# LIS-TU-Berlin/SVN-ICP

Measured on AMD Instinct MI355X. Metric: scan-pair registrations/sec at N particles x M source pts, 1/2/4/8 GPU, higher is better.
Workload: dtype f64; 1 GPU; C3: 128 particles SVN-ICP, 131072-pt source vs 262144-pt target, K=100, I=20, max_dist=1.0, lr=1.0, SVNFullGrad=False, correspondence=fast, early stop off; synthetic 64-beam scans (seed 20250718); particles=128, target_points=262144, knn_count=100, parallelism=single GPU

## Files before the change

svn-icp_amd/csrc/particle_update.hip:

```cpp
#include "kernels.hpp"
#include "update_single.hpp"
#include "stein_split_device.hpp"

namespace svnicp {

namespace {

constexpr int UT = 512;
constexpr int KREG = 32;

struct Work {
  double *H, *b, *N, *x, *phi, *sq;
  __device__ Work(double* w, int P) {
    H = w; b = H + (size_t)P * 36; N = b + (size_t)P * 6; x = N + (size_t)P * 6; phi = x + (size_t)P * 6;
    sq = phi + (size_t)P * 6;
  }
};

__device__ __forceinline__ void load_sums(const UpdateArgs& a, int p, double* s) {
  const double* rec = a.sums + (size_t)p * kNSums;
  const size_t stride = a.sums_stride ? (size_t)a.sums_stride : (size_t)a.P * kNSums;
#pragma unroll
  for (int i = 0; i < kNSums; ++i) s[i] = rec[i];
  for (int r = 1; r < a.n_ranks; ++r) {
// ... 1249 lines not shown
    r[0] = init[3 * P + p]; r[1] = init[4 * P + p]; r[2] = init[5 * P + p];
    tv[0] = init[p]; tv[1] = init[P + p]; tv[2] = init[2 * P + p];
    if (mode == 0) so3_exp(r, Rm, nullptr); else euler_to_R(r[0], r[1], r[2], Rm);
    if (mode == 1 && eul) {
      for (int i = 0; i < 3; ++i) { eul[6 * p + i] = tv[i]; eul[6 * p + 3 + i] = r[i]; }
    }
  }
  double Rt[9], tt[3];
  mat3_mul(pose.R0, Rm, Rt);
  mat3_vec(pose.R0, tv, tt);
  for (int i = 0; i < 9; ++i) { R[9 * p + i] = Rm[i]; Rtot[12 * p + i] = Rt[i]; }
  for (int i = 0; i < 3; ++i) { t[3 * p + i] = tv[i]; Rtot[12 * p + 9 + i] = pose.t0[i] + tt[i]; }
  if (refresh_pose) {
    double lg[3];
    if (mode == 0) so3_log(Rm, lg); else { lg[0] = r[0]; lg[1] = r[1]; lg[2] = r[2]; }
    for (int i = 0; i < 3; ++i) { pose_out[i * P + p] = tv[i]; pose_out[(3 + i) * P + p] = lg[i]; }
  }
}

__global__ void k_stats(StatsArgs a) {
  const int tid = threadIdx.x;
  const int P = a.P;
  __shared__ double mean[6];
  constexpr int kStage = 1024;
  __shared__ double sp[6 * kStage];
  const bool staged = P <= kStage;
  if (staged) for (int e = tid; e < 6 * P; e += blockDim.x) sp[e] = a.pose[e];
  __syncthreads();
  const double* pose = staged ? sp : a.pose;
  const double wsvn = (double)(1.0f / (float)P);
  if (tid < 6) {
    double s = 0.0;
    if (a.mode == 0) { for (int p = 0; p < P; ++p) s += pose[tid * P + p] * wsvn; }
    else { for (int p = 0; p < P; ++p) s += pose[tid * P + p]; s /= P; }
    mean[tid] = s;
    a.out[tid] = s;
  }
  __syncthreads();
  if (tid < 6) {
    double s = 0.0;
    if (a.mode == 0) { for (int p = 0; p < P; ++p) { const double d = pose[tid * P + p] - mean[tid]; s += d * d * wsvn; } }
    else { for (int p = 0; p < P; ++p) { const double d = pose[tid * P + p] - mean[tid]; s += d * d; } s /= (P - 1); }
    a.out[6 + tid] = s;
  }
  if (tid < 36) {
    const int r = tid / 6, c = tid % 6;
    double s = 0.0;
    const double wgt = a.mode == 0 ? wsvn : 1.0;
    for (int p = 0; p < P; ++p) s += wgt * ((pose[r * P + p] - mean[r]) * (pose[c * P + p] - mean[c]));
    a.out[12 + tid] = a.mode == 0 ? s : s / P;
  }
  for (int p = tid; p < P; p += blockDim.x) a.out[48 + p] = a.mode == 0 ? wsvn : 1.0;
}

}

size_t update_workspace_doubles(int P) { return (size_t)P * (36 + 6 * 4) + (size_t)P * P + 64; }
size_t update_uctl_doubles(int P) { return (size_t)UCTL_NORM + (size_t)((P + 7) & ~7) + (size_t)HB_NB / 2 + (size_t)36 * ((P + 127) / 128) + 8; }

hipError_t launch_init_particles(const double* init6xP, int P, const Pose0& pose, int mode, double* R, double* t,
                                 double* Rtot, double* pose_out, int refresh_pose, double* eul, hipStream_t st, const BeginZero* zero) {
  BeginZero z{};
  if (zero) z = *zero;
  unsigned int most = 0;
  for (int a = 0; a < z.n; ++a) most = z.dwords[a] > most ? z.dwords[a] : most;
  int blocks = (P + 127) / 128;
  const int for_zero = (int)((most + 128u * 32u - 1u) / (128u * 32u));
  if (for_zero > blocks) blocks = for_zero > 256 ? 256 : for_zero;
  hipLaunchKernelGGL(k_init_particles, dim3(blocks), dim3(128), 0, st, init6xP, P, pose, mode, R, t, Rtot,
                     pose_out, refresh_pose, eul, z);
  return hipGetLastError();
}

hipError_t launch_update_median(const UpdateArgs& a, int num_cus, int max_p_one_workgroup, hipStream_t st) {
  const int P = a.P;
  if (P <= max_p_one_workgroup && P <= 128) {
    const size_t smem = (size_t)P * 6 * sizeof(double) + (size_t)(FRONT_BUF + 8) * sizeof(double) + (size_t)HB_NB * sizeof(unsigned int);
    hipError_t e = hipFuncSetAttribute(reinterpret_cast<const void*>(k_upd_median), hipFuncAttributeMaxDynamicSharedMemorySize, (int)smem);
    if (e != hipSuccess) return e;
    hipLaunchKernelGGL(k_upd_median, dim3(1), dim3(UT), smem, st, a);
    return hipGetLastError();
  }
  const size_t n = (size_t)P * P;
  const size_t xs = (size_t)P * 6 * sizeof(double);
  int nb = (int)((n + 1023) / 1024);
  if (nb > num_cus / 2) nb = num_cus / 2;
  if (nb < 1) nb = 1;
  const size_t lds_hist = xs + (size_t)HB_NB * sizeof(unsigned int);
  const size_t lds_coll = xs + (size_t)COLL_CHUNK * sizeof(double);
  const size_t lds_sel = (size_t)SEL_LDS_KEYS * sizeof(double);
  if (lds_hist > 150 * 1024 || lds_coll > 150 * 1024) return hipErrorInvalidValue;
  {
    hipError_t e = hipFuncSetAttribute(reinterpret_cast<const void*>(k_upd_hist), hipFuncAttributeMaxDynamicSharedMemorySize, 150 * 1024);
    if (e == hipSuccess) e = hipFuncSetAttribute(reinterpret_cast<const void*>(k_upd_collect), hipFuncAttributeMaxDynamicSharedMemorySize, 150 * 1024);
    if (e == hipSuccess) e = hipFuncSetAttribute(reinterpret_cast<const void*>(k_upd_select), hipFuncAttributeMaxDynamicSharedMemorySize, (int)lds_sel);
    if (e != hipSuccess) return e;
  }
  hipLaunchKernelGGL(k_upd_hist, dim3(nb), dim3(256), lds_hist, st, a);
  hipLaunchKernelGGL(k_upd_collect, dim3(nb), dim3(256), lds_coll, st, a);
  hipLaunchKernelGGL(k_upd_select, dim3(1), dim3(UT), lds_sel, st, a);
  return hipGetLastError();
}

hipError_t launch_update_prepare(const UpdateArgs& a, hipStream_t st) {
  const int need_mean = (!a.svgd && !a.full_grad) ? 1 : 0;
  hipLaunchKernelGGL(k_upd_prepare, dim3((a.P + PREP_PW - 1) / PREP_PW + need_mean), dim3(PREP_T), 0, st, a);
  return hipGetLastError();
}

hipError_t launch_update_prepare_median(const UpdateArgs& a, hipStream_t st) {
  const int P = a.P;
  const int need_mean = (!a.svgd && !a.full_grad) ? 1 : 0;
  const size_t smem = (size_t)P * 6 * sizeof(double) + (size_t)(FRONT_BUF + 8) * sizeof(double) + (size_t)HB_NB * sizeof(unsigned int);
  hipError_t e = hipFuncSetAttribute(reinterpret_cast<const void*>(k_upd_prepare_median), hipFuncAttributeMaxDynamicSharedMemorySize, (int)smem);
  if (e != hipSuccess) return e;
  hipLaunchKernelGGL(k_upd_prepare_median, dim3((P + PREP_PW - 1) / PREP_PW + need_mean + 1), dim3(UT), smem, st, a);
  return hipGetLastError();
}

namespace {
template <int PW, int WP, int NRB, bool TAIL>
hipError_t launch_small_t(const AccumArgs& a, const UpdateArgs& u, const SmallArgs& s, int grid, size_t smem, hipStream_t st) {
  const void* fn = u.svgd ? reinterpret_cast<const void*>(k_small_registration<PW, WP, NRB, TAIL, true>)
                          : reinterpret_cast<const void*>(k_small_registration<PW, WP, NRB, TAIL, false>);
  hipError_t e = hipFuncSetAttribute(fn, hipFuncAttributeMaxDynamicSharedMemorySize, (int)smem);
  if (e != hipSuccess) return e;
  int per_cu = 0;
  e = hipOccupancyMaxActiveBlocksPerMultiprocessor(&per_cu, fn, 256, smem);
  if (e != hipSuccess) return e;
  if (per_cu < 1) return hipErrorCooperativeLaunchTooLarge;
  AccumArgs aa = a; UpdateArgs uu = u; SmallArgs ss = s;
  void* args[3] = {&aa, &uu, &ss};
  return hipLaunchCooperativeKernel(fn, dim3((unsigned)grid), dim3(256), args, (unsigned int)smem, st);
}
}

bool small_registration_supported(int PW, int WP, int K) {
  return K >= 97 && K <= 100 && ((WP == 1 && (PW == 16 || PW == 32 || PW == 64)) || (PW == 64 && WP == 2));
}

hipError_t launch_small_registration(const AccumPlan& plan, AccumArgs a, const UpdateArgs& u, int iterations, unsigned int* bar,
                                     int num_cus, hipStream_t st) {
  const int P = u.P;
  a.Ppad = plan.Ppad; a.pts_per_block = plan.pts_per_block; a.spts_per_block = plan.pts_per_block;
  SmallArgs s{};
  s.GA = plan.grid_x; s.iterations = iterations; s.bar = bar;
  {
    const int pass = 4 * (64 / plan.PW);
    int64_t spb = (a.B + (num_cus - 2)) / (num_cus - 1);
    spb = (spb + pass - 1) / pass * pass;
    s.spts_per_block = (int)spb;
    s.GS = (int)((a.B + spb - 1) / spb);
  }
  const int n_prep = (P + PREP_PW - 1) / PREP_PW + ((!u.svgd && !u.full_grad) ? 1 : 0);
  const int n_dir = (P + 3) / 4;
  int grid = s.GS + 1;
  if (s.GA > grid) grid = s.GA;
  if (n_prep > grid) grid = n_prep;
  if (n_dir > grid) grid = n_dir;
  if (grid > num_cus) return hipErrorCooperativeLaunchTooLarge;
  const size_t smem_median = (size_t)P * 6 * sizeof(double) + (size_t)(FRONT_BUF + 8) * sizeof(double) + (size_t)HB_NB * sizeof(unsigned int);
  const size_t smem = smem_median > plan.smem ? smem_median : plan.smem;
  if (!small_registration_supported(plan.PW, plan.WP, plan.K)) return hipErrorInvalidValue;
  if (plan.PW == 16) return launch_small_t<16, 1, 6, true>(a, u, s, grid, smem, st);
  if (plan.PW == 32) return launch_small_t<32, 1, 6, true>(a, u, s, grid, smem, st);
  if (plan.WP == 1) return launch_small_t<64, 1, 6, true>(a, u, s, grid, smem, st);
  return launch_small_t<64, 2, 6, true>(a, u, s, grid, smem, st);
}

hipError_t launch_update_direction(const UpdateArgs& a, hipStream_t st, bool finish) {
  hipLaunchKernelGGL(k_upd_direction, dim3((a.P + 3) / 4), dim3(256), 0, st, a);
  if (finish && (a.check_early_stop || a.trH)) hipLaunchKernelGGL(k_upd_finish, dim3(1), dim3(256), 0, st, a);
  return hipGetLastError();
}
const double* update_step_norms(const UpdateArgs& a) { return a.uctl + UCTL_NORM; }

hipError_t launch_reduce_partials(const double* partial, int nblk, int Ppad, int p_lo, int n_particles, double* sums, const int* ctl,
                                  hipStream_t st) {
  const int n_entries = n_particles * kNSums;
  if (n_entries <= 0) return hipSuccess;
  hipLaunchKernelGGL(k_reduce_partials, dim3((n_entries + 15) / 16), dim3(256), 0, st, partial, nblk, Ppad, p_lo, n_particles, sums, ctl);
  return hipGetLastError();
}

hipError_t launch_update(const UpdateArgs& a_in, hipStream_t st) {
  UpdateArgs a = a_in;
  const size_t base = (size_t)a.P * 24 * sizeof(double);
  const size_t with_h = base + (size_t)a.P * 36 * sizeof(double);
  a.h_in_lds = with_h <= 120 * 1024 ? 1 : 0;
  const size_t smem = a.h_in_lds ? with_h : base;
  if (smem > 150 * 1024) return hipErrorInvalidValue;
  if (smem > 64 * 1024) {
    hipError_t e = hipFuncSetAttribute(reinterpret_cast<const void*>(k_particle_update),
                                       hipFuncAttributeMaxDynamicSharedMemorySize, (int)smem);
    if (e != hipSuccess) return e;
  }
  hipLaunchKernelGGL(k_particle_update, dim3(1), dim3(UT), smem, st, a);
  return hipGetLastError();
}

hipError_t launch_update_svgd(const UpdateArgs& a, hipStream_t st) {
  const size_t smem = (size_t)a.P * 18 * sizeof(double);
  if (smem > 150 * 1024) return hipErrorInvalidValue;
  if (smem > 64 * 1024) {
    hipError_t e = hipFuncSetAttribute(reinterpret_cast<const void*>(k_particle_update_svgd),
                                       hipFuncAttributeMaxDynamicSharedMemorySize, (int)smem);
    if (e != hipSuccess) return e;
  }
  hipLaunchKernelGGL(k_particle_update_svgd, dim3(1), dim3(UT), smem, st, a);
  return hipGetLastError();
}

hipError_t launch_stats(const StatsArgs& a, hipStream_t st) {
  hipLaunchKernelGGL(k_stats, dim3(1), dim3(256), 0, st, a);
  return hipGetLastError();
}

}
```

svn-icp_amd/csrc/stein_split.hip:

```cpp
#include "stein_split_device.hpp"

namespace svnicp {

namespace {

constexpr float kSentinelCC = 1.0e30f;
__global__ __launch_bounds__(256) void k_build_table3(const int32_t* __restrict__ idx, int64_t B, int K,
                                                      const double* __restrict__ tgt, int64_t M, double* __restrict__ table,
                                                      double* __restrict__ anchor, float4* __restrict__ tablea,
                                                      float* __restrict__ cmax) {
  __shared__ float rowbuf[4][128 * 4];
  const int lane = threadIdx.x & (kWave - 1), wave = threadIdx.x >> 6;
  const int64_t b = (int64_t)blockIdx.x * 4 + wave;
  if (b >= B) return;
  int64_t i0 = idx[b * K];
  i0 = i0 < 0 ? 0 : (i0 >= M ? M - 1 : i0);
  const double a0 = tgt[3 * i0], a1 = tgt[3 * i0 + 1], a2 = tgt[3 * i0 + 2];
  float cm = 0.0f;
  float* rb = rowbuf[wave];
  for (int k = lane; k < 128; k += kWave) {
    float cx = 0.f, cy = 0.f, cz = 0.f, cc = kSentinelCC;
    if (k < K) {
      int64_t i = idx[b * K + k];
      i = i < 0 ? 0 : (i >= M ? M - 1 : i);
      const double x = tgt[3 * i], y = tgt[3 * i + 1], z = tgt[3 * i + 2];
      if (table) {
        double* o = table + ((size_t)b * K + k) * 3;
        o[0] = x; o[1] = y; o[2] = z;
      }
      cx = (float)(x - a0); cy = (float)(y - a1); cz = (float)(z - a2);
      cc = (float)(((double)cx * cx + (double)cy * cy) + (double)cz * cz);
      cm = __builtin_fmaxf(cm, (float)sqrt(((double)cx * cx + (double)cy * cy) + (double)cz * cz) * 1.0000002f);
      if (!(cc < kSentinelCC)) cm = __builtin_nanf("");
    }
    rb[4 * k] = cx; rb[4 * k + 1] = cy; rb[4 * k + 2] = cz; rb[4 * k + 3] = cc;
  }
  for (int off = 32; off > 0; off >>= 1) {
    const float o = __shfl_xor(cm, off, kWave);
    cm = (cm != cm || o != o) ? __builtin_nanf("") : __builtin_fmaxf(cm, o);
  }
  if (lane == 0) {
    cmax[b] = cm;
    anchor[3 * b] = a0; anchor[3 * b + 1] = a1; anchor[3 * b + 2] = a2;
  }
  __builtin_amdgcn_wave_barrier();
  const int mi = lane & 15, mk = lane >> 4;
#pragma unroll
  for (int h = 0; h < 2; ++h) {
    float4 v;
    v.x = rb[4 * (16 * (4 * h + 0) + mi) + mk];
    v.y = rb[4 * (16 * (4 * h + 1) + mi) + mk];
    v.z = rb[4 * (16 * (4 * h + 2) + mi) + mk];
    v.w = rb[4 * (16 * (4 * h + 3) + mi) + mk];
    tablea[((size_t)b * 2 + h) * 64 + lane] = v;
  }
}


inline int row_code_for(int K) { return K <= 16 ? 1 : K <= 32 ? 2 : K <= 64 ? 4 : K <= 96 ? 6 : K <= 100 ? 60 : K <= 112 ? 7 : 8; }

template <int PW, int WP, int NRB, bool TAIL>
hipError_t launch_s(const AccumPlan& plan, const AccumArgs& a, hipStream_t st) {
  hipLaunchKernelGGL((k_stein_search_bf16<PW, WP, NRB, TAIL>), dim3(plan.sgrid_x, plan.grid_y), dim3(NT), 0, st, a);
  return hipGetLastError();
}
template <int PW, int WP>
hipError_t launch_srb(const AccumPlan& plan, const AccumArgs& a, hipStream_t st) {
  switch (row_code_for(a.K)) {
    case 1: return launch_s<PW, WP, 1, false>(plan, a, st);
    case 2: return launch_s<PW, WP, 2, false>(plan, a, st);
    case 4: return launch_s<PW, WP, 4, false>(plan, a, st);
    case 6: return launch_s<PW, WP, 6, false>(plan, a, st);
    case 60: return launch_s<PW, WP, 6, true>(plan, a, st);
    case 7: return launch_s<PW, WP, 7, false>(plan, a, st);
    default: return launch_s<PW, WP, 8, false>(plan, a, st);
  }
}
template <int PW, int WP>
hipError_t launch_w(const AccumPlan& plan, const AccumArgs& a, hipStream_t st) {
  if (!a.svgd && !a.corr && !a.full_idx) hipLaunchKernelGGL((k_stein_accumulate_w<PW, WP, true>), dim3(plan.grid_x, plan.grid_y), dim3(NT), plan.smem, st, a);
  else if (a.svgd && !a.corr && !a.full_idx) hipLaunchKernelGGL((k_stein_accumulate_w<PW, WP, true, true>), dim3(plan.grid_x, plan.grid_y), dim3(NT), plan.smem, st, a);
  else hipLaunchKernelGGL((k_stein_accumulate_w<PW, WP, false>), dim3(plan.grid_x, plan.grid_y), dim3(NT), plan.smem, st, a);
  return hipGetLastError();
}

template <int PW, int WP, int NRB, bool TAIL>
hipError_t occ_search(int* n) {
  return hipOccupancyMaxActiveBlocksPerMultiprocessor(n, k_stein_search_bf16<PW, WP, NRB, TAIL>, NT, 0);
}
template <int PW, int WP>
void occ_split(int K, size_t smem, int* search, int* accum) {
  int n = 0;
  hipError_t e;
  switch (row_code_for(K)) {
    case 1: e = occ_search<PW, WP, 1, false>(&n); break;
    case 2: e = occ_search<PW, WP, 2, false>(&n); break;
    case 4: e = occ_search<PW, WP, 4, false>(&n); break;
    case 6: e = occ_search<PW, WP, 6, false>(&n); break;
    case 60: e = occ_search<PW, WP, 6, true>(&n); break;
    case 7: e = occ_search<PW, WP, 7, false>(&n); break;
    default: e = occ_search<PW, WP, 8, false>(&n); break;
  }
  *search = (e != hipSuccess || n < 1) ? 4 : (n > 8 ? 8 : n);
  n = 0;
  e = hipOccupancyMaxActiveBlocksPerMultiprocessor(&n, k_stein_accumulate_w<PW, WP, true>, NT, smem);
  *accum = (e != hipSuccess || n < 1) ? 3 : (n > 8 ? 8 : n);
}

}

void split_occupancy_blocks(int PW, int WP, int K, size_t smem, int* search, int* accum) {
  switch (PW) {
    case 16: return occ_split<16, 1>(K, smem, search, accum);
    case 32: return occ_split<32, 1>(K, smem, search, accum);
    default:
      if (WP == 1) return occ_split<64, 1>(K, smem, search, accum);
      if (WP == 2) return occ_split<64, 2>(K, smem, search, accum);
      return occ_split<64, 4>(K, smem, search, accum);
  }
}

hipError_t launch_build_table3(const int32_t* idx, int64_t B, int K, const double* tgt, int64_t M, double* table,
                               double* anchor, float4* tablea, float* cmax, hipStream_t st) {
  if (B <= 0) return hipSuccess;
  hipLaunchKernelGGL(k_build_table3, dim3((unsigned)((B + 3) / 4)), dim3(256), 0, st, idx, B, K, tgt, M, table, anchor, tablea,
                     cmax);
  return hipGetLastError();
}


hipError_t launch_search_split(const AccumPlan& plan, AccumArgs a, hipStream_t st) {
  a.Ppad = plan.Ppad; a.pts_per_block = plan.pts_per_block; a.spts_per_block = plan.spts_per_block;
  switch (plan.PW) {
    case 16: return launch_srb<16, 1>(plan, a, st);
    case 32: return launch_srb<32, 1>(plan, a, st);
    default:
      if (plan.WP == 1) return launch_srb<64, 1>(plan, a, st);
      if (plan.WP == 2) return launch_srb<64, 2>(plan, a, st);
      return launch_srb<64, 4>(plan, a, st);
  }
}

__global__ __launch_bounds__(256) void k_transform_cloud(const double* __restrict__ src, int64_t B, const double* __restrict__ pose12,
                                                         double* __restrict__ q, const int* __restrict__ ctl) {
  if (ctl[0]) return;
  const int64_t b = (int64_t)blockIdx.x * blockDim.x + threadIdx.x;
  if (b >= B) return;
  const double s0 = src[3 * b], s1 = src[3 * b + 1], s2 = src[3 * b + 2];
  q[3 * b] = (s0 * pose12[0] + s1 * pose12[1] + s2 * pose12[2]) + pose12[9];
  q[3 * b + 1] = (s0 * pose12[3] + s1 * pose12[4] + s2 * pose12[5]) + pose12[10];
  q[3 * b + 2] = (s0 * pose12[6] + s1 * pose12[7] + s2 * pose12[8]) + pose12[11];
}

hipError_t launch_transform_cloud(const double* src, int64_t B, const double* pose12, double* q, const int* ctl, hipStream_t st) {
  if (B <= 0) return hipSuccess;
  hipLaunchKernelGGL(k_transform_cloud, dim3((unsigned)((B + 255) / 256)), dim3(256), 0, st, src, B, pose12, q, ctl);
  return hipGetLastError();
}

hipError_t launch_accumulate_split(const AccumPlan& plan, const AccumArgs& a, hipStream_t st) {
  switch (plan.PW) {
    case 16: return launch_w<16, 1>(plan, a, st);
    case 32: return launch_w<32, 1>(plan, a, st);
    default:
      if (plan.WP == 1) return launch_w<64, 1>(plan, a, st);
      if (plan.WP == 2) return launch_w<64, 2>(plan, a, st);
      return launch_w<64, 4>(plan, a, st);
  }
}

}
```

svn-icp_amd/csrc/stein_split_device.hpp:

```cpp
#pragma once
#include <cstdlib>
#include "kernels.hpp"
#include "stein_common.hpp"

namespace svnicp {

namespace {

typedef float v4f __attribute__((ext_vector_type(4)));
#define SVNICP_CONST_AS __attribute__((address_space(4)))

__device__ __forceinline__ float pack_slot(float v, unsigned int mask, unsigned int bits) {
  return __uint_as_float((__float_as_uint(v) & ~mask) | bits);
}
__device__ __forceinline__ float imin_f(float a, float b) {
  const int x = (int)__float_as_uint(a), y = (int)__float_as_uint(b);
  return __uint_as_float((unsigned int)(x < y ? x : y));
}
__device__ __forceinline__ float imax_f(float a, float b) {
  const int x = (int)__float_as_uint(a), y = (int)__float_as_uint(b);
  return __uint_as_float((unsigned int)(x > y ? x : y));
}

typedef __bf16 bf2 __attribute__((ext_vector_type(2)));
typedef float f2v __attribute__((ext_vector_type(2)));
typedef __bf16 bf8 __attribute__((ext_vector_type(8)));
typedef unsigned int u4v __attribute__((ext_vector_type(4)));

__device__ __forceinline__ unsigned int cvt_pk_bf16(float lo, float hi) {
  const f2v v = {lo, hi};
  return __builtin_bit_cast(unsigned int, __builtin_convertvector(v, bf2));
}
__device__ __forceinline__ bf8 split_a3(float x) {
  const unsigned int r0 = cvt_pk_bf16(x, x);
  const float e1 = x - __uint_as_float(r0 & 0xffff0000u);
  const unsigned int r1 = cvt_pk_bf16(x, e1);
  const float e2 = e1 - __uint_as_float(r1 & 0xffff0000u);
  const unsigned int r2 = cvt_pk_bf16(e1, e2);
  const u4v t = {r0, r1, r2, r2};
  return __builtin_bit_cast(bf8, t);
}
__device__ __forceinline__ bf8 split_b3(float x) {
  const unsigned int r0 = cvt_pk_bf16(x, x);
  const float e1 = x - __uint_as_float(r0 & 0xffff0000u);
  const unsigned int q0 = cvt_pk_bf16(x, e1);
  const float e2 = e1 - __uint_as_float(q0 & 0xffff0000u);
  const unsigned int q1 = cvt_pk_bf16(e2, x);
  const unsigned int q2 = cvt_pk_bf16(e1, x);
  const u4v t = {q0, q1, q2, 0u};
  return __builtin_bit_cast(bf8, t);
}
__device__ __forceinline__ float pack_slot3(float v, unsigned int bits) {
  return __uint_as_float(__builtin_amdgcn_bitop3_b32(__float_as_uint(v), 31u, bits, 0xBA));
}
__device__ __forceinline__ float fmin_raw(float a, float b) { return __builtin_elementwise_minimum(a, b); }
__device__ __forceinline__ float fmax_raw(float a, float b) { return __builtin_elementwise_maximum(a, b); }
__device__ __forceinline__ float fmed3_raw(float a, float b, float c) { return __builtin_amdgcn_fmed3f(a, b, c); }
__device__ __forceinline__ float fmin3_raw(float a, float b, float c) { return __builtin_elementwise_minimum(__builtin_elementwise_minimum(a, b), c); }
constexpr int kQueueCap = 1024;

template <int G>
__device__ __forceinline__ int exact_nearest_of_k(const AccumArgs& a, const double (*pose)[64], int64_t b, int pl, int K, int sub) {
  constexpr int NIT = 128 / G;
  const double* sp = a.src + 3 * b;
  const int32_t* ci = a.cand + (size_t)b * K;
  int64_t ti[NIT];
#pragma unroll
  for (int i = 0; i < NIT; ++i) {
    const int k = sub + i * G;
    int64_t t = ci[k < K ? k : 0];
    ti[i] = t < 0 ? 0 : (t >= a.M ? a.M - 1 : t);
  }
  double rx[NIT], ry[NIT], rz[NIT];
#pragma unroll
  for (int i = 0; i < NIT; ++i) {
    const double* r = a.tgt + 3 * ti[i];
    rx[i] = r[0]; ry[i] = r[1]; rz[i] = r[2];
  }
  const double u0 = sp[0], u1 = sp[1], u2 = sp[2];
  const double t0 = (u0 * pose[0][pl] + u1 * pose[1][pl] + u2 * pose[2][pl]) + pose[9][pl];
  const double t1 = (u0 * pose[3][pl] + u1 * pose[4][pl] + u2 * pose[5][pl]) + pose[10][pl];
  const double t2 = (u0 * pose[6][pl] + u1 * pose[7][pl] + u2 * pose[8][pl]) + pose[11][pl];
  double bd = __builtin_huge_val(), d_first = 0.0;
  int bk = 0x7fffffff;
#pragma unroll
  for (int i = 0; i < NIT; ++i) {
    const int k = sub + i * G;
    const double dx = t0 - rx[i], dy = t1 - ry[i], dz = t2 - rz[i];
    const double d = (dx * dx + dy * dy) + dz * dz;
    if (k == 0) d_first = d;
    if (k < K && (d < bd || (d == bd && k < bk))) { bd = d; bk = k; }
  }
#pragma unroll
  for (int off = G / 2; off > 0; off >>= 1) {
    const double od = __shfl_xor(bd, off, kWave);
    const int ok = __shfl_xor(bk, off, kWave);
    if (od < bd || (od == bd && ok < bk)) { bd = od; bk = ok; }
  }
  const double d0 = __shfl(d_first, (threadIdx.x & (kWave - 1)) & ~(G - 1), kWave);
  return (d0 != d0 || bk == 0x7fffffff) ? 0 : bk;
}

#ifndef SVNICP_SEARCH_EPS_U
#define SVNICP_SEARCH_EPS_U 54
#endif
constexpr float kEpsBf16 = (float)SVNICP_SEARCH_EPS_U * 5.9604644775390625e-08f;

#ifndef SVNICP_SEARCH_WAVES
#define SVNICP_SEARCH_WAVES 4
#endif
template <int PW, int WP, int NRB, bool TAIL>
__device__ __forceinline__ void search_body(const AccumArgs& a, int bx, int by) {
  if (a.ctl[0]) return;
  if (a.fin_iteration >= 0 && bx == 0 && by == 0) {
    __shared__ double sh_fin[NT];
    __shared__ int sh_fin_stop;
    const int ftid = threadIdx.x, FP = a.fin_P;
    double fs = 0.0;
    for (int p = ftid; p < FP; p += NT) fs += a.fin_norms[p];
    sh_fin[ftid] = fs;
    __syncthreads();
    for (int off = NT / 2; off > 0; off >>= 1) {
      if (ftid < off) sh_fin[ftid] += sh_fin[ftid + off];
      __syncthreads();
    }
    if (ftid == 0) {
      const double m = sh_fin[0] / FP;
      const int stop = (float)m < (float)a.fin_thr;
      if (stop) { a.fin_ctl[0] = 1; a.fin_ctl[1] = a.fin_iteration + 1; }
      sh_fin_stop = stop;
    }
    __syncthreads();
    if (sh_fin_stop) return;
    for (int e = ftid; e < 6 * FP; e += NT) a.fin_history[(size_t)a.fin_iteration * 6 * FP + e] = (float)a.fin_pose[e];
  }
  constexpr int BW = kWave / PW;
  constexpr int CBP = PW / 16;
  constexpr int NPT = 4 / CBP;
  constexpr int ST = 4 * BW;
  constexpr bool PIPE = NPT == 1;
  constexpr int NTILE = 4 * NRB + (TAIL ? 1 : 0);
  __shared__ float4 s_rows[4][NPT][4][NTILE];
  __shared__ float4 s_scr4[4][64];
  __shared__ double s_pose[WP][12][64];
  __shared__ unsigned int s_queue[kQueueCap];
  __shared__ unsigned int s_qn, s_qsteps;
  const int tid = threadIdx.x;
  if (tid == 0) { s_qn = 0u; s_qsteps = 0u; }
#pragma unroll
  for (int i = 0; i < kQueueCap / NT; ++i) s_queue[tid + i * NT] = 0xffffffffu;
  const int lane = tid & (kWave - 1);
  const int wave = __builtin_amdgcn_readfirstlane(tid >> 6);
  const int pl = lane % PW, bs = lane / PW;
  const int mj = lane & 15, mk = lane >> 4;
  const int pbase = by * (WP * PW);
  for (int g = wave; g < WP; g += 4) {
    const int p = a.p_lo + pbase + g * PW + pl;
    const double* rp = a.Rtot + 12 * (size_t)(p < a.p_hi ? p : a.p_lo);
#pragma unroll
    for (int i = 0; i < 12; ++i) s_pose[g][i][lane] = rp[i];
  }
  const int K = a.K;
  const SVNICP_CONST_AS v4f* ctab = (const SVNICP_CONST_AS v4f*)a.tablea;
  float* const rows_w = reinterpret_cast<float*>(&s_rows[wave][0][mj & 3][mj >> 2]) + mk;
  const int64_t blk_lo = (int64_t)bx * a.spts_per_block;
  const int64_t blk_hi = (blk_lo + a.spts_per_block < a.B) ? blk_lo + a.spts_per_block : a.B;
  __syncthreads();
  const int64_t nfirst = blk_lo + wave * BW;

  int pend_idx = 0;
  size_t pend_off = 0;
  bool pend_have = false;
  v4f alo_n, ahi_n;
  double sa_n = 0.0;
  float c_n = 0.0f;
  auto fetch_point = [&](int64_t nn) {
    const double* base = lane < 3 ? a.src + 3 * nn : a.anchor + 3 * nn - 3;
    sa_n = base[lane < 6 ? lane : 3];
    c_n = a.cmax[nn];
  };
  v4f ralo_n[PIPE ? 1 : NPT], rahi_n[PIPE ? 1 : NPT];
  auto fetch_rows = [&](int64_t n0, int pt) {
    int64_t bq = n0 + pt;
    bq = bq < blk_hi ? bq : (n0 < blk_hi ? n0 : blk_lo);
    const SVNICP_CONST_AS v4f* rowp = ctab + (size_t)bq * 128 + lane;
    ralo_n[pt] = rowp[0];
    rahi_n[pt] = ralo_n[pt];
    if constexpr (NRB > 4) rahi_n[pt] = rowp[64];
  };
  if constexpr (!PIPE) {
#pragma unroll
    for (int pt = 0; pt < NPT; ++pt) fetch_rows(nfirst, pt);
  }
  if constexpr (PIPE) {
    fetch_point(nfirst < blk_hi ? nfirst : blk_lo);
    const SVNICP_CONST_AS v4f* rowp = ctab + (size_t)(nfirst < blk_hi ? nfirst : blk_lo) * 128 + lane;
    alo_n = rowp[0];
    ahi_n = alo_n;
    if constexpr (NRB > 4) ahi_n = rowp[64];
  }

  for (int64_t n = nfirst; n < blk_hi; n += ST) {
    const int64_t b = n + bs;
    const bool inb = b < blk_hi;
    double s0, s1, s2, a0, a1, a2;
    float C;
    if constexpr (PIPE) {
      s0 = rdlane_f64(sa_n, 0); s1 = rdlane_f64(sa_n, 1); s2 = rdlane_f64(sa_n, 2);
      a0 = rdlane_f64(sa_n, 3); a1 = rdlane_f64(sa_n, 4); a2 = rdlane_f64(sa_n, 5);
      C = __uint_as_float((unsigned int)__builtin_amdgcn_readfirstlane((int)__float_as_uint(c_n)));
    } else {
      const int64_t bl = inb ? b : n;
      const double* sp = a.src + 3 * bl;
      const double* an = a.anchor + 3 * bl;
      s0 = sp[0]; s1 = sp[1]; s2 = sp[2];
      a0 = an[0]; a1 = an[1]; a2 = an[2];
      C = a.cmax[bl];
    }

    bf8 afr[NRB];
    auto split_rows = [&](v4f alo, v4f ahi, int pt) {
#pragma unroll
      for (int rb = 0; rb < NRB; ++rb) {
        const float v = rb == 0 ? alo.x : rb == 1 ? alo.y : rb == 2 ? alo.z : rb == 3 ? alo.w
                      : rb == 4 ? ahi.x : rb == 5 ? ahi.y : rb == 6 ? ahi.z : ahi.w;
        afr[rb] = split_a3(v);
        rows_w[(pt * 4 * NTILE + 4 * rb) * 4] = v;
      }
      if constexpr (TAIL) {
        const float v = NRB == 4 ? ahi.x : NRB == 5 ? ahi.y : NRB == 6 ? ahi.z : ahi.w;
        if (mj < 4) rows_w[(pt * 4 * NTILE + 4 * NRB) * 4] = v;
      }
    };
    if constexpr (PIPE) {
      const v4f alo = alo_n, ahi = ahi_n;
      int64_t nn = n + ST;
      nn = nn < blk_hi ? nn : n;
      const SVNICP_CONST_AS v4f* rowp = ctab + (size_t)nn * 128 + lane;
      alo_n = rowp[0];
      if constexpr (NRB > 4) ahi_n = rowp[64];
      fetch_point(nn);
      __builtin_amdgcn_wave_barrier();
      split_rows(alo, ahi, 0);
    }

#pragma nounroll
    for (int g = 0; g < WP; ++g) {
      float E, mm0, mm1, mm2;
      {
        const double (*pose)[64] = s_pose[g];
        const double T0 = (s0 * pose[0][lane] + s1 * pose[1][lane] + s2 * pose[2][lane]) + pose[9][lane];
        const double T1 = (s0 * pose[3][lane] + s1 * pose[4][lane] + s2 * pose[5][lane]) + pose[10][lane];
        const double T2 = (s0 * pose[6][lane] + s1 * pose[7][lane] + s2 * pose[8][lane]) + pose[11][lane];
        const float xf0 = (float)(T0 - a0), xf1 = (float)(T1 - a1), xf2 = (float)(T2 - a2);
        const float X2 = __builtin_amdgcn_sqrtf(__builtin_fmaf(xf0, xf0, __builtin_fmaf(xf1, xf1, xf2 * xf2))) * 1.000002f;
        const float Cq = __builtin_fmaf(5.9604644775390625e-08f, X2, C);
        E = kEpsBf16 * Cq * __builtin_fmaf(2.0f, X2, Cq);
        mm0 = -2.0f * xf0; mm1 = -2.0f * xf1; mm2 = -2.0f * xf2;
        if (g > 0) __builtin_amdgcn_wave_barrier();
        s_scr4[wave][lane] = make_float4(mm0, mm1, mm2, 1.0f);
        __builtin_amdgcn_wave_barrier();
      }
      const float* scr4f = reinterpret_cast<const float*>(s_scr4[wave]);
      float b1[4], b2[4];
      float braw[4];
#pragma unroll
      for (int cb = 0; cb < 4; ++cb) braw[cb] = scr4f[(16 * cb + mj) * 4 + mk];

#pragma unroll
      for (int cb = 0; cb < 4; ++cb) {
        if constexpr (!PIPE) {
          if (cb % CBP == 0) {
            split_rows(ralo_n[cb / CBP], rahi_n[cb / CBP], cb / CBP);
            fetch_rows(n + ST, cb / CBP);
          }
        }
        const bf8 bfr = split_b3(braw[cb]);
        const v4f zero = {0.0f, 0.0f, 0.0f, 0.0f};
        float m1 = 0.0f, m2 = 0.0f, wp = 0.0f, rp = 0.0f, pend0 = 0.0f, pend1 = 0.0f;
        int np = 0;
        bool have_m = false;
        bool have_p = false;
        v4f dcur = __builtin_amdgcn_mfma_f32_16x16x32_bf16(afr[0], bfr, zero, 0, 0, 0);
#pragma unroll
        for (int rb = 0; rb < NRB; ++rb) {
          v4f dnext = dcur;
          if (rb + 1 < NRB) dnext = __builtin_amdgcn_mfma_f32_16x16x32_bf16(afr[rb + 1], bfr, zero, 0, 0, 0);
          const float pk = pack_slot3(fmin_raw(fmin3_raw(dcur[0], dcur[1], dcur[2]), dcur[3]), (unsigned int)rb);
          if (np == 0) { pend0 = pk; np = 1; }
          else if (np == 1) { pend1 = pk; np = 2; }
          else {
            np = 0;
            const float w = fmin3_raw(pend0, pend1, pk), r = fmed3_raw(pend0, pend1, pk);
            if (!have_p) { wp = w; rp = r; have_p = true; }
            else {
              have_p = false;
              if (!have_m) {
                m1 = fmin_raw(wp, w);
                m2 = fmin3_raw(fmax_raw(wp, w), rp, r);
                have_m = true;
              } else {
                const float md = fmed3_raw(m1, wp, w);
                m2 = fmin_raw(fmin3_raw(m2, rp, r), md);
                m1 = fmin3_raw(m1, wp, w);
              }
            }
          }
          dcur = dnext;
        }
        if (!have_m) { m1 = __builtin_huge_valf(); m2 = __builtin_huge_valf(); }
        if (have_p) { const float t = fmax_raw(m1, wp); m1 = fmin_raw(m1, wp); m2 = fmin3_raw(t, m2, rp); }
        if (np >= 1) { m2 = fmed3_raw(m1, m2, pend0); m1 = fmin_raw(m1, pend0); }
        if (np >= 2) { m2 = fmed3_raw(m1, m2, pend1); m1 = fmin_raw(m1, pend1); }
        b1[cb] = m1; b2[cb] = m2;
      }
#pragma unroll
      for (int cb = 0; cb < 4; ++cb) b1[cb] = __uint_as_float(__builtin_amdgcn_bitop3_b32(__float_as_uint(b1[cb]), 0x18u, (unsigned int)mk << 3, 0xBA));
      auto merge2 = [&](float p1, float q1, float p2, float q2, float& o1, float& o2) {
        o1 = fmin_raw(p1, q1);
        o2 = fmin_raw(fmax_raw(p1, q1), fmin_raw(p2, q2));
      };
      float b1own, b2own;
      {
        float h1[2], h2[2];
#pragma unroll
        for (int j = 0; j < 2; ++j) {
          const auto r1 = __builtin_amdgcn_permlane16_swap(__float_as_uint(b1[2 * j]), __float_as_uint(b1[2 * j + 1]), false, false);
          const auto r2 = __builtin_amdgcn_permlane16_swap(__float_as_uint(b2[2 * j]), __float_as_uint(b2[2 * j + 1]), false, false);
          merge2(__uint_as_float(r1[0]), __uint_as_float(r1[1]), __uint_as_float(r2[0]), __uint_as_float(r2[1]), h1[j], h2[j]);
        }
        const auto r1 = __builtin_amdgcn_permlane32_swap(__float_as_uint(h1[0]), __float_as_uint(h1[1]), false, false);
        const auto r2 = __builtin_amdgcn_permlane32_swap(__float_as_uint(h2[0]), __float_as_uint(h2[1]), false, false);
        merge2(__uint_as_float(r1[0]), __uint_as_float(r1[1]), __uint_as_float(r2[0]), __uint_as_float(r2[1]), b1own, b2own);
      }
      if constexpr (TAIL) {
        const float4* tl = &s_rows[wave][bs][0][4 * NRB];
        float sc[4];
#pragma unroll
        for (int t = 0; t < 4; ++t) {
          const float4 c = tl[t * NTILE];
          sc[t] = __builtin_fmaf(c.x, mm0, __builtin_fmaf(c.y, mm1, __builtin_fmaf(c.z, mm2, c.w)));
        }
        const float pk = pack_slot(fmin_raw(fmin3_raw(sc[0], sc[1], sc[2]), sc[3]), 0x1fu, (unsigned int)NRB);
        b2own = fmed3_raw(b1own, b2own, pk);
        b1own = fmin_raw(b1own, pk);
      }

      const int pin = g * PW + pl;
      const bool valid = inb && (a.p_lo + pbase + pin) < a.p_hi;
      const unsigned int wbits = __float_as_uint(b1own);
      int tile = (int)(((wbits & 7u) << 2) | ((wbits >> 3) & 3u));
      tile = tile < NTILE ? tile : NTILE - 1;
      const float thr = 2.0f * E + 3.83e-06f * (__builtin_fabsf(b1own) + __builtin_fabsf(b2own)) + 1.0e-30f;
      const bool tiles_ok = b2own - b1own > thr;
      float pk4[4];
      {
        const float4* rt = &s_rows[wave][bs][0][tile];
        if constexpr (!PIPE) __builtin_amdgcn_wave_barrier();
#pragma unroll
        for (int t = 0; t < 4; ++t) {
          const float4 r = rt[t * NTILE];
          const float sc = __builtin_fmaf(r.x, mm0, __builtin_fmaf(r.y, mm1, __builtin_fmaf(r.z, mm2, r.w)));
          pk4[t] = __uint_as_float(__builtin_amdgcn_bitop3_b32(__float_as_uint(sc), 3u, (unsigned int)t, 0xBA));
        }
      }
      const float w3 = fmin3_raw(pk4[0], pk4[1], pk4[2]), r3 = fmed3_raw(pk4[0], pk4[1], pk4[2]);
      const float v1 = fmin_raw(w3, pk4[3]), v2 = fmed3_raw(w3, r3, pk4[3]);
      const float thrv = 2.0f * E + 4.76837158203125e-07f * (__builtin_fabsf(v1) + __builtin_fabsf(v2)) + 1.0e-30f;
      int kb = 4 * tile + (int)(__float_as_uint(v1) & 3u);
      const bool ambiguous = valid && (!tiles_ok || !(v2 - v1 > thrv) || kb >= K);
      kb = kb < K ? kb : 0;
      unsigned long long am = __ballot(ambiguous);
      if (am) {
        const int cnt = __builtin_popcountll(am);
        int base = 0;
        if (lane == 0) { base = (int)atomicAdd(&s_qn, (unsigned int)cnt); atomicAdd(&s_qsteps, 1u); }
        base = __builtin_amdgcn_readfirstlane(base);
        if (base + cnt <= kQueueCap) {
          if (ambiguous) {
            const int rank = __builtin_popcountll(am & ((1ull << lane) - 1ull));
            s_queue[base + rank] = ((unsigned int)(b - blk_lo) << 8) | (unsigned int)pin;
          }
        } else {
          do {
            const int L = (int)__builtin_ctzll(am);
            am &= am - 1;
            const int ke = exact_nearest_of_k<kWave>(a, s_pose[g], n + L / PW, L % PW, K, lane);
            if (lane == L) kb = ke;
          } while (am);
        }
      }
      if (pend_have) a.kidx[pend_off] = pend_idx;
      pend_have = inb;
      if (inb) {
        pend_off = (size_t)b * a.Ppad + (pbase + pin);
        a.kbest[pend_off] = (uint8_t)kb;
        pend_idx = a.cand[(size_t)b * K + kb];
      }
    }
    __builtin_amdgcn_wave_barrier();
  }

  if (pend_have) a.kidx[pend_off] = pend_idx;
  __syncthreads();
  {
    const unsigned int total = s_qn < (unsigned int)kQueueCap ? s_qn : (unsigned int)kQueueCap;
    constexpr int kExactLanes = 32;
    const int sub = lane & (kExactLanes - 1);
    for (unsigned int e = (unsigned int)(tid / kExactLanes); e < total; e += NT / kExactLanes) {
      const unsigned int ent = s_queue[e];
      if (ent == 0xffffffffu) continue;
      const int64_t be = blk_lo + (int64_t)(ent >> 8);
      const int pin = (int)(ent & 0xffu);
      const int ke = exact_nearest_of_k<kExactLanes>(a, s_pose[pin / PW], be, pin % PW, K, sub);
      if (sub == 0) {
        a.kbest[(size_t)be * a.Ppad + (pbase + pin)] = (uint8_t)ke;
        a.kidx[(size_t)be * a.Ppad + (pbase + pin)] = a.cand[(size_t)be * K + ke];
      }
    }
    if (tid == 0 && a.ambig_count && s_qsteps) { atomicAdd(a.ambig_count, (int)s_qsteps); atomicAdd(a.ambig_count + 1, (int)s_qn); }
  }
}

template <int PW, int WP, int NRB, bool TAIL>
__global__ __launch_bounds__(NT, (PW == 16 || WP == 4) ? 3 : SVNICP_SEARCH_WAVES) void k_stein_search_bf16(AccumArgs a) {
  search_body<PW, WP, NRB, TAIL>(a, xcd_block((int)blockIdx.x, (int)gridDim.x), (int)blockIdx.y);
}

template <int PW, int WP, bool PLAIN, bool SVGD = false>
__device__ __forceinline__ void accumulate_body(const AccumArgs& a, int bx, int by, double* lds) {
  if (a.ctl[0]) return;
  constexpr int BW = kWave / PW;
  constexpr int WB = 4 / WP;
#ifndef SVNICP_ACCUM_U
#define SVNICP_ACCUM_U 4
#endif
  constexpr int U = SVNICP_ACCUM_U;
  const int tid = threadIdx.x;
  const int lane = tid & (kWave - 1);
  const int wave = __builtin_amdgcn_readfirstlane(tid >> 6);
  const int wp = wave % WP, wb = wave / WP;
  const int pl = lane % PW, bs = lane / PW;
  const int pidx = by * (WP * PW) + wp * PW + pl;
  const int p = a.p_lo + pidx;
  const bool pvalid = p < a.p_hi;

  double Rt[9], tt[3];
  {
    const double* rp = a.Rtot + 12 * (size_t)(pvalid ? p : a.p_lo);
#pragma unroll
    for (int i = 0; i < 9; ++i) Rt[i] = rp[i];
#pragma unroll
    for (int i = 0; i < 3; ++i) tt[i] = rp[9 + i];
  }
  double acc[kNSums];
#pragma unroll
  for (int i = 0; i < kNSums; ++i) acc[i] = 0.0;
  const int K = a.K;
  const int64_t blk_lo = (int64_t)bx * a.pts_per_block;
  const int64_t blk_hi = (blk_lo + a.pts_per_block < a.B) ? blk_lo + a.pts_per_block : a.B;
  constexpr int STEP = WB * BW;
  const SVNICP_CONST_AS double* csrc = (const SVNICP_CONST_AS double*)a.src;
  const SVNICP_CONST_AS int32_t* ccand = (const SVNICP_CONST_AS int32_t*)a.cand;
  const SVNICP_CONST_AS double* ctgt = (const SVNICP_CONST_AS double*)a.tgt;
  const uint8_t* kbp = a.kbest + pidx;
  const int32_t* kip = a.kidx + pidx;

  const int32_t* fullp = (!PLAIN && a.full_idx) ? a.full_idx + (size_t)(pvalid ? p : a.p_lo) * a.B : nullptr;
  auto load_kb = [&](int64_t n) -> int {
    const int64_t b = n + bs;
    const int64_t bc = b < blk_hi ? b : blk_lo;
    if (PLAIN) return kip[(size_t)bc * a.Ppad];
    if (fullp) return fullp[bc];
    return (int)kbp[(size_t)bc * a.Ppad];
  };
  const double c3d = 3.0 / a.max_dist;
  auto accumulate = [&](double on, double s0, double s1, double s2, double q0, double q1, double q2) {
    const double T0 = (s0 * Rt[0] + s1 * Rt[1] + s2 * Rt[2]) + tt[0];
    const double T1 = (s0 * Rt[3] + s1 * Rt[4] + s2 * Rt[5]) + tt[1];
    const double T2 = (s0 * Rt[6] + s1 * Rt[7] + s2 * Rt[8]) + tt[2];
    const double dx = T0 - q0, dy = T1 - q1, dz = T2 - q2;
    const double best = (dx * dx + dy * dy) + dz * dz;
    const double mf = best < a.max_dist ? on : 0.0;
    const double x = mf * best;
    const double r0 = __builtin_amdgcn_rsq(x + 0x1p-1000);
    const double sa = x * r0, h0 = 0.5 * r0;
    const double ea = fma(-h0, sa, 0.5);
    const double sb = fma(sa, ea, sa);
    const double nn = fma(fma(-sb, sb, x), h0, sb);
    const double den = fma(c3d, nn, 1.0);
    const double y0 = __builtin_amdgcn_rcp(den);
    const double y1 = fma(y0, fma(-den, y0, 1.0), y0);
    const double wq = fma(y1, fma(-den, y1, 1.0), y1);
    const double w = on * (wq * wq);
    const double we = mf * w;
    const double e0 = we * dx, e1 = we * dy, e2 = we * dz;
    const double w0 = we * s0, w1 = we * s1, w2 = we * s2;
    acc[0] += w;
    acc[1] += w0; acc[2] += w1; acc[3] += w2;
    if (PLAIN ? SVGD : (a.svgd != 0)) acc[4] += (((T0 + T1) + T2) != 0.0) ? mf : 0.0;
    else acc[4] = fma(w0, s0, acc[4]);
    acc[5] = fma(w0, s1, acc[5]); acc[6] = fma(w0, s2, acc[6]);
    acc[7] = fma(w1, s1, acc[7]); acc[8] = fma(w1, s2, acc[8]); acc[9] = fma(w2, s2, acc[9]);
    acc[10] += e0; acc[11] += e1; acc[12] += e2;
    acc[13] = fma(e0, s0, acc[13]); acc[14] = fma(e0, s1, acc[14]); acc[15] = fma(e0, s2, acc[15]);
    acc[16] = fma(e1, s0, acc[16]); acc[17] = fma(e1, s1, acc[17]); acc[18] = fma(e1, s2, acc[18]);
    acc[19] = fma(e2, s0, acc[19]); acc[20] = fma(e2, s1, acc[20]); acc[21] = fma(e2, s2, acc[21]);
  };

  const int64_t n0 = blk_lo + wb * BW;
  int kbn[U];
#pragma unroll
  for (int u = 0; u < U; ++u) kbn[u] = load_kb(n0 + u * STEP);
  for (int64_t n = n0; n < blk_hi; n += U * STEP) {
    int kb[U];
    int64_t ti[U];
#pragma unroll
    for (int u = 0; u < U; ++u) {
      kb[u] = kbn[u];
      const int64_t b = n + u * STEP + bs;
      const int64_t bl = b < blk_hi ? b : blk_lo;
      const int64_t t = (PLAIN || fullp) ? (int64_t)kb[u] : (int64_t)ccand[(size_t)bl * K + kb[u]];
      ti[u] = t < 0 ? 0 : (t >= a.M ? a.M - 1 : t);
    }
#pragma unroll
    for (int u = 0; u < U; ++u) kbn[u] = load_kb(n + (U + u) * STEP);
    double q[U][3];
#pragma unroll
    for (int u = 0; u < U; ++u) {
      const SVNICP_CONST_AS double* r = ctgt + 3 * ti[u];
      q[u][0] = r[0]; q[u][1] = r[1]; q[u][2] = r[2];
    }
#pragma unroll
    for (int u = 0; u < U; ++u) {
      const int64_t b = n + u * STEP + bs;
      const bool valid = pvalid && b < blk_hi;
      const int64_t bl = b < blk_hi ? b : blk_lo;
      const SVNICP_CONST_AS double* sp = csrc + 3 * bl;
      const double s0 = sp[0], s1 = sp[1], s2 = sp[2];
      if (!PLAIN && a.corr && valid) a.corr[(size_t)p * a.B + b] = kb[u];
      accumulate(b < blk_hi ? 1.0 : 0.0, s0, s1, s2, q[u][0], q[u][1], q[u][2]);
    }
  }

#pragma unroll
  for (int off = PW; off < kWave; off <<= 1) {
#pragma unroll
    for (int i = 0; i < kNSums; ++i) acc[i] += __shfl_xor(acc[i], off, kWave);
  }
  if constexpr (WB > 1) {
    double* red = lds;
    if (wb > 0 && bs == 0) {
      double* r = red + ((size_t)(wb - 1) * (WP * PW) + wp * PW + pl) * kNSums;
#pragma unroll
      for (int i = 0; i < kNSums; ++i) r[i] = acc[i];
    }
// ... 25 lines not shown
```

Measured before the change: 142.3 registrations/s.

## Pad search row tiles, deepen MFMA pipeline, and use 32-bit pair offsets

Changes the shared-memory row layout in the bf16 nearest-neighbour search kernel to a padded, odd-multiple stride so the transpose writes and tile reads avoid bank conflicts, and simplifies slot packing so the tile index is taken directly from the low bits. It issues MFMAs two row-blocks ahead instead of one to hide matrix latency, restructures the bf16 three-way split, and computes kbest/kidx/cand addresses with 32-bit offsets from a per-step row base to cut 64-bit address arithmetic. A host-side bound check rejects launches where those 32-bit offsets could overflow. Out-of-range kb now clamps to K-1 instead of 0, and the deeper MFMA prefetch adds register pressure.

```diff
diff --git a/svn-icp_amd/csrc/particle_update.hip b/svn-icp_amd/csrc/particle_update.hip
--- a/svn-icp_amd/csrc/particle_update.hip
+++ b/svn-icp_amd/csrc/particle_update.hip
@@ -1425,6 +1425,7 @@
     s.spts_per_block = (int)spb;
     s.GS = (int)((a.B + spb - 1) / spb);
   }
+  if (!search_offsets_fit(a.Ppad, a.K)) return hipErrorInvalidValue;
   const int n_prep = (P + PREP_PW - 1) / PREP_PW + ((!u.svgd && !u.full_grad) ? 1 : 0);
   const int n_dir = (P + 3) / 4;
   int grid = s.GS + 1;
diff --git a/svn-icp_amd/csrc/search_limits.hpp b/svn-icp_amd/csrc/search_limits.hpp
--- /dev/null
+++ b/svn-icp_amd/csrc/search_limits.hpp
@@ -0,0 +1,13 @@
+#pragma once
+#include <cstdint>
+
+namespace svnicp {
+
+constexpr int64_t kSearchPointsPerStep = 4;
+
+constexpr int64_t search_offset_bound(int Ppad, int K) {
+  return 4 * kSearchPointsPerStep * (int64_t)(Ppad > K ? Ppad : K);
+}
+constexpr bool search_offsets_fit(int Ppad, int K) { return search_offset_bound(Ppad, K) <= ((int64_t)1 << 32); }
+
+}
diff --git a/svn-icp_amd/csrc/stein_split.hip b/svn-icp_amd/csrc/stein_split.hip
--- a/svn-icp_amd/csrc/stein_split.hip
+++ b/svn-icp_amd/csrc/stein_split.hip
@@ -131,6 +131,7 @@
 
 hipError_t launch_search_split(const AccumPlan& plan, AccumArgs a, hipStream_t st) {
   a.Ppad = plan.Ppad; a.pts_per_block = plan.pts_per_block; a.spts_per_block = plan.spts_per_block;
+  if (!search_offsets_fit(a.Ppad, a.K)) return hipErrorInvalidValue;
   switch (plan.PW) {
     case 16: return launch_srb<16, 1>(plan, a, st);
     case 32: return launch_srb<32, 1>(plan, a, st);
diff --git a/svn-icp_amd/csrc/stein_split_device.hpp b/svn-icp_amd/csrc/stein_split_device.hpp
--- a/svn-icp_amd/csrc/stein_split_device.hpp
+++ b/svn-icp_amd/csrc/stein_split_device.hpp
@@ -2,6 +2,7 @@
 #include <cstdlib>
 #include "kernels.hpp"
 #include "stein_common.hpp"
+#include "search_limits.hpp"
 
 namespace svnicp {
 
@@ -41,10 +42,9 @@
   return __builtin_bit_cast(bf8, t);
 }
 __device__ __forceinline__ bf8 split_b3(float x) {
-  const unsigned int r0 = cvt_pk_bf16(x, x);
-  const float e1 = x - __uint_as_float(r0 & 0xffff0000u);
+  const float e1 = x - __uint_as_float(cvt_pk_bf16(0.0f, x));
+  const float e2 = e1 - __uint_as_float(cvt_pk_bf16(0.0f, e1));
   const unsigned int q0 = cvt_pk_bf16(x, e1);
-  const float e2 = e1 - __uint_as_float(q0 & 0xffff0000u);
   const unsigned int q1 = cvt_pk_bf16(e2, x);
   const unsigned int q2 = cvt_pk_bf16(e1, x);
   const u4v t = {q0, q1, q2, 0u};
@@ -140,7 +140,8 @@
   constexpr int ST = 4 * BW;
   constexpr bool PIPE = NPT == 1;
   constexpr int NTILE = 4 * NRB + (TAIL ? 1 : 0);
-  __shared__ float4 s_rows[4][NPT][4][NTILE];
+  constexpr int RS = 16 * (((4 * NTILE + 15) / 16) | 1);
+  __shared__ float4 s_rows[4][NPT][4][RS / 4];
   __shared__ float4 s_scr4[4][64];
   __shared__ double s_pose[WP][12][64];
   __shared__ unsigned int s_queue[kQueueCap];
@@ -162,14 +163,16 @@
   }
   const int K = a.K;
   const SVNICP_CONST_AS v4f* ctab = (const SVNICP_CONST_AS v4f*)a.tablea;
-  float* const rows_w = reinterpret_cast<float*>(&s_rows[wave][0][mj & 3][mj >> 2]) + mk;
+  float* const rows_w = reinterpret_cast<float*>(&s_rows[wave][0][mk][0]) + mj;
   const int64_t blk_lo = (int64_t)bx * a.spts_per_block;
   const int64_t blk_hi = (blk_lo + a.spts_per_block < a.B) ? blk_lo + a.spts_per_block : a.B;
+  static_assert(BW <= kSearchPointsPerStep, "search_limits.hpp bounds the pair offsets for at most this many points per step");
   __syncthreads();
   const int64_t nfirst = blk_lo + wave * BW;
 
   int pend_idx = 0;
-  size_t pend_off = 0;
+  int32_t* pend_row = a.kidx;
+  unsigned int pend_off4 = 0;
   bool pend_have = false;
   v4f alo_n, ahi_n;
   double sa_n = 0.0;
@@ -225,11 +228,11 @@
         const float v = rb == 0 ? alo.x : rb == 1 ? alo.y : rb == 2 ? alo.z : rb == 3 ? alo.w
                       : rb == 4 ? ahi.x : rb == 5 ? ahi.y : rb == 6 ? ahi.z : ahi.w;
         afr[rb] = split_a3(v);
-        rows_w[(pt * 4 * NTILE + 4 * rb) * 4] = v;
+        rows_w[pt * 4 * RS + 16 * rb] = v;
       }
       if constexpr (TAIL) {
         const float v = NRB == 4 ? ahi.x : NRB == 5 ? ahi.y : NRB == 6 ? ahi.z : ahi.w;
-        if (mj < 4) rows_w[(pt * 4 * NTILE + 4 * NRB) * 4] = v;
+        if (mj < 4) rows_w[pt * 4 * RS + 16 * NRB] = v;
       }
     };
     if constexpr (PIPE) {
@@ -282,11 +285,13 @@
         bool have_m = false;
         bool have_p = false;
         v4f dcur = __builtin_amdgcn_mfma_f32_16x16x32_bf16(afr[0], bfr, zero, 0, 0, 0);
+        v4f dnext = dcur;
+        if (NRB > 1) dnext = __builtin_amdgcn_mfma_f32_16x16x32_bf16(afr[NRB > 1 ? 1 : 0], bfr, zero, 0, 0, 0);
 #pragma unroll
         for (int rb = 0; rb < NRB; ++rb) {
-          v4f dnext = dcur;
-          if (rb + 1 < NRB) dnext = __builtin_amdgcn_mfma_f32_16x16x32_bf16(afr[rb + 1], bfr, zero, 0, 0, 0);
-          const float pk = pack_slot3(fmin_raw(fmin3_raw(dcur[0], dcur[1], dcur[2]), dcur[3]), (unsigned int)rb);
+          v4f dn2 = dnext;
+          if (rb + 2 < NRB) dn2 = __builtin_amdgcn_mfma_f32_16x16x32_bf16(afr[rb + 2 < NRB ? rb + 2 : 0], bfr, zero, 0, 0, 0);
+          const float pk = pack_slot3(fmin_raw(fmin3_raw(dcur[0], dcur[1], dcur[2]), dcur[3]), 4u * rb);
           if (np == 0) { pend0 = pk; np = 1; }
           else if (np == 1) { pend1 = pk; np = 2; }
           else {
@@ -306,7 +311,7 @@
               }
             }
           }
-          dcur = dnext;
+          dcur = dnext; dnext = dn2;
         }
         if (!have_m) { m1 = __builtin_huge_valf(); m2 = __builtin_huge_valf(); }
         if (have_p) { const float t = fmax_raw(m1, wp); m1 = fmin_raw(m1, wp); m2 = fmin3_raw(t, m2, rp); }
@@ -315,7 +320,7 @@
         b1[cb] = m1; b2[cb] = m2;
       }
 #pragma unroll
-      for (int cb = 0; cb < 4; ++cb) b1[cb] = __uint_as_float(__builtin_amdgcn_bitop3_b32(__float_as_uint(b1[cb]), 0x18u, (unsigned int)mk << 3, 0xBA));
+      for (int cb = 0; cb < 4; ++cb) b1[cb] = __uint_as_float(__builtin_amdgcn_bitop3_b32(__float_as_uint(b1[cb]), 3u, (unsigned int)mk, 0xBA));
       auto merge2 = [&](float p1, float q1, float p2, float q2, float& o1, float& o2) {
         o1 = fmin_raw(p1, q1);
         o2 = fmin_raw(fmax_raw(p1, q1), fmin_raw(p2, q2));
@@ -333,43 +338,42 @@
         const auto r2 = __builtin_amdgcn_permlane32_swap(__float_as_uint(h2[0]), __float_as_uint(h2[1]), false, false);
         merge2(__uint_as_float(r1[0]), __uint_as_float(r1[1]), __uint_as_float(r2[0]), __uint_as_float(r2[1]), b1own, b2own);
       }
+      auto score_tile = [&](int tile, float* sc) {
+        const float4 cx = s_rows[wave][bs][0][tile], cy = s_rows[wave][bs][1][tile];
+        const float4 cz = s_rows[wave][bs][2][tile], cc = s_rows[wave][bs][3][tile];
+        sc[0] = __builtin_fmaf(cx.x, mm0, __builtin_fmaf(cy.x, mm1, __builtin_fmaf(cz.x, mm2, cc.x)));
+        sc[1] = __builtin_fmaf(cx.y, mm0, __builtin_fmaf(cy.y, mm1, __builtin_fmaf(cz.y, mm2, cc.y)));
+        sc[2] = __builtin_fmaf(cx.z, mm0, __builtin_fmaf(cy.z, mm1, __builtin_fmaf(cz.z, mm2, cc.z)));
+        sc[3] = __builtin_fmaf(cx.w, mm0, __builtin_fmaf(cy.w, mm1, __builtin_fmaf(cz.w, mm2, cc.w)));
+      };
       if constexpr (TAIL) {
-        const float4* tl = &s_rows[wave][bs][0][4 * NRB];
         float sc[4];
-#pragma unroll
-        for (int t = 0; t < 4; ++t) {
-          const float4 c = tl[t * NTILE];
-          sc[t] = __builtin_fmaf(c.x, mm0, __builtin_fmaf(c.y, mm1, __builtin_fmaf(c.z, mm2, c.w)));
-        }
-        const float pk = pack_slot(fmin_raw(fmin3_raw(sc[0], sc[1], sc[2]), sc[3]), 0x1fu, (unsigned int)NRB);
+        score_tile(4 * NRB, sc);
+        const float pk = pack_slot3(fmin_raw(fmin3_raw(sc[0], sc[1], sc[2]), sc[3]), 4u * NRB);
         b2own = fmed3_raw(b1own, b2own, pk);
         b1own = fmin_raw(b1own, pk);
       }
 
       const int pin = g * PW + pl;
       const bool valid = inb && (a.p_lo + pbase + pin) < a.p_hi;
-      const unsigned int wbits = __float_as_uint(b1own);
-      int tile = (int)(((wbits & 7u) << 2) | ((wbits >> 3) & 3u));
+      int tile = (int)(__float_as_uint(b1own) & 31u);
       tile = tile < NTILE ? tile : NTILE - 1;
       const float thr = 2.0f * E + 3.83e-06f * (__builtin_fabsf(b1own) + __builtin_fabsf(b2own)) + 1.0e-30f;
       const bool tiles_ok = b2own - b1own > thr;
       float pk4[4];
       {
-        const float4* rt = &s_rows[wave][bs][0][tile];
         if constexpr (!PIPE) __builtin_amdgcn_wave_barrier();
-#pragma unroll
-        for (int t = 0; t < 4; ++t) {
-          const float4 r = rt[t * NTILE];
-          const float sc = __builtin_fmaf(r.x, mm0, __builtin_fmaf(r.y, mm1, __builtin_fmaf(r.z, mm2, r.w)));
-          pk4[t] = __uint_as_float(__builtin_amdgcn_bitop3_b32(__float_as_uint(sc), 3u, (unsigned int)t, 0xBA));
-        }
+        float sc[4];
+        score_tile(tile, sc);
+#pragma unroll
+        for (int t = 0; t < 4; ++t) pk4[t] = __uint_as_float(__builtin_amdgcn_bitop3_b32(__float_as_uint(sc[t]), 3u, (unsigned int)t, 0xBA));
       }
       const float w3 = fmin3_raw(pk4[0], pk4[1], pk4[2]), r3 = fmed3_raw(pk4[0], pk4[1], pk4[2]);
       const float v1 = fmin_raw(w3, pk4[3]), v2 = fmed3_raw(w3, r3, pk4[3]);
       const float thrv = 2.0f * E + 4.76837158203125e-07f * (__builtin_fabsf(v1) + __builtin_fabsf(v2)) + 1.0e-30f;
       int kb = 4 * tile + (int)(__float_as_uint(v1) & 3u);
-      const bool ambiguous = valid && (!tiles_ok || !(v2 - v1 > thrv) || kb >= K);
-      kb = kb < K ? kb : 0;
+      const bool ambiguous = valid & (!tiles_ok | !(v2 - v1 > thrv) | (kb >= K));
+      kb = kb < K ? kb : K - 1;
       unsigned long long am = __ballot(ambiguous);
       if (am) {
         const int cnt = __builtin_popcountll(am);
@@ -390,18 +394,21 @@
           } while (am);
         }
       }
-      if (pend_have) a.kidx[pend_off] = pend_idx;
+      if (pend_have) *(int32_t*)((char*)pend_row + pend_off4) = pend_idx;
       pend_have = inb;
+      pend_row = a.kidx + n * a.Ppad + pbase;
       if (inb) {
-        pend_off = (size_t)b * a.Ppad + (pbase + pin);
-        a.kbest[pend_off] = (uint8_t)kb;
-        pend_idx = a.cand[(size_t)b * K + kb];
+        const unsigned int bl = (unsigned int)bs;
+        const unsigned int off = bl * (unsigned int)a.Ppad + (unsigned int)pin;
+        (a.kbest + n * a.Ppad + pbase)[off] = (uint8_t)kb;
+        pend_off4 = 4u * off;
+        pend_idx = *(const int32_t*)((const char*)(a.cand + n * K) + 4u * (bl * (unsigned int)K + (unsigned int)kb));
       }
     }
     __builtin_amdgcn_wave_barrier();
   }
 
-  if (pend_have) a.kidx[pend_off] = pend_idx;
+  if (pend_have) *(int32_t*)((char*)pend_row + pend_off4) = pend_idx;
   __syncthreads();
   {
     const unsigned int total = s_qn < (unsigned int)kQueueCap ? s_qn : (unsigned int)kQueueCap;
```

New measurement: 144.6 registrations/s, median of 6. +1.7%, better.
